# salute-developers/GigaAM

Hardware: AMD Instinct MI355X
Metric: RTFx v2_ctc batch32x20s (log-mel + encoder + greedy decode) (higher is better)
Workload: dtype f32 (GEMMs: 3-term split on fp16 MFMA, fp32 accumulate)

## Files before the change

### gigaam_amd/_lib.py

```python
from __future__ import annotations

import ctypes as C
import os
from typing import Optional

_HERE = os.path.dirname(os.path.abspath(__file__))
LIB_NAME = "libgigaam_hip.so"
LIB_PATH = os.path.join(_HERE, LIB_NAME)

SUBS_CONV2D, SUBS_CONV1D = 0, 1
ATT_ROTARY, ATT_REL_POS = 0, 1
NORM_BATCH, NORM_LAYER = 0, 1
HEAD_NONE, HEAD_CTC, HEAD_RNNT, HEAD_EMO = 0, 1, 2, 3
DTYPE_F32, DTYPE_F16, DTYPE_BF16, DTYPE_F64, DTYPE_I64 = 0, 1, 2, 3, 4
GEMM_F32, GEMM_F16X3, GEMM_F16 = 0, 1, 2
PF_CLASSES = ["gemm", "conv2", "attn", "norm", "convmod", "stem", "frontend", "decode", "misc", "align_bt", "align_out"]


class GamConfig(C.Structure):
    _fields_ = [(n, C.c_int32) for n in (
        "sample_rate", "n_mels", "hop_length", "win_length", "n_fft", "center",
        "feat_in", "n_layers", "d_model", "subsampling", "subs_kernel_size", "subsampling_factor",
        "ff_expansion_factor", "self_attention_model", "n_heads", "pos_emb_max_len",
        "conv_norm_type", "conv_kernel_size",
        "head_type", "num_classes", "pred_hidden", "pred_rnn_layers", "joint_hidden",
    )]


_P = C.c_void_p
SIGNATURES = {
    "gam_abi_version": (C.c_int, []),
    "gam_create": (C.c_int, [C.POINTER(GamConfig), C.c_int, C.POINTER(_P)]),
    "gam_destroy": (None, [_P]),
    "gam_set_weight": (C.c_int, [_P, C.c_char_p, _P, C.c_int, C.POINTER(C.c_int64), C.c_int]),
    "gam_finalize": (C.c_int, [_P]),
    "gam_feat_frames": (C.c_int64, [_P, C.c_int64]),
    "gam_enc_frames": (C.c_int64, [_P, C.c_int64]),
    "gam_frontend": (C.c_int, [_P, _P, _P, C.c_int, C.c_int64, _P, _P, _P]),
    "gam_encode": (C.c_int, [_P, _P, _P, C.c_int, C.c_int64, _P, _P, _P]),
    "gam_encode_ex": (C.c_int, [_P, _P, _P, C.c_int, C.c_int64, _P, _P, C.c_int, _P, _P]),
    "gam_encode_varlen": (C.c_int, [_P, _P, _P, C.POINTER(C.c_int64), C.c_int, C.c_int64, _P, _P, C.c_int, _P, _P]),
    "gam_last_encode_rows": (C.c_int, [_P, C.POINTER(C.c_int)]),
    "gam_ctc_head": (C.c_int, [_P, _P, C.c_int, C.c_int64, _P, _P]),
    "gam_ctc_greedy": (C.c_int, [_P, _P, _P, C.c_int, C.c_int64, _P, _P, _P, _P]),
    "gam_ctc_align": (C.c_int, [_P, _P, _P, C.c_int, C.c_int64, _P, _P, C.c_int, _P, _P, _P, _P, _P, _P, _P]),
    "gam_op_ctc_align": (C.c_int, [_P, _P, _P, C.c_int, C.c_int64, C.c_int, _P, _P, C.c_int, _P, _P, _P, _P, _P, _P, _P]),
    "gam_op_ctc_align_long": (C.c_int, [_P, _P, C.c_int64, C.c_int, _P, C.c_int, _P, _P, _P, _P, _P, _P, _P]),
    "gam_set_ctc_align_workspace": (C.c_int, [_P, C.c_int64]),
    "gam_tune_ctc_align_long": (C.c_int, [C.c_int, C.c_int]),
    "gam_ctc_kws": (C.c_int, [_P, _P, _P, C.c_int, C.c_int64, C.c_int, _P, _P, _P, _P, _P, _P]),
    "gam_op_ctc_kws": (C.c_int, [_P, _P, _P, C.c_int, C.c_int64, C.c_int, C.c_int, _P, _P, _P, _P, _P, _P]),
    "gam_set_keywords": (C.c_int, [_P, _P, _P, C.c_int, _P]),
    "gam_ctc_beam": (C.c_int, [_P, _P, _P, C.c_int, C.c_int64, C.c_int, _P, _P, _P, _P, _P, _P]),
    "gam_op_ctc_beam": (C.c_int, [_P, _P, _P, C.c_int, C.c_int64, C.c_int, C.c_int, _P, _P, _P, _P, _P, _P]),
    "gam_set_hotwords": (C.c_int, [_P, _P, _P, C.c_int, C.c_float]),
    "gam_set_lm": (C.c_int, [_P, _P, C.c_int, _P, C.c_int64, C.c_int, _P, C.c_int64, C.c_int, C.c_int, C.c_int, C.c_int, C.c_int,
                             C.c_float, C.c_float, C.c_float]),
    "gam_rnnt_greedy": (C.c_int, [_P, _P, _P, C.c_int, C.c_int64, C.c_int, _P, _P, _P, _P, _P, C.c_int, _P]),
    "gam_ctc_beam_nbest": (C.c_int, [_P, _P, _P, C.c_int, C.c_int64, C.c_int, C.c_int, _P, _P, _P, _P, _P, _P, _P]),
    "gam_op_ctc_beam_nbest": (C.c_int, [_P, _P, _P, C.c_int, C.c_int64, C.c_int, C.c_int, C.c_int, _P, _P, _P, _P, _P, _P, _P]),
    "gam_rnnt_beam_nbest": (C.c_int, [_P, _P, _P, C.c_int, C.c_int64, C.c_int, C.c_int, C.c_int, _P, _P, _P, _P, _P, _P, _P]),
    "gam_op_rnnt_beam_nbest": (C.c_int, [_P, _P, _P, C.c_int, C.c_int64, C.c_int, C.c_int, C.c_int, _P, _P, _P, _P, _P, _P, _P]),
    "gam_rnnt_beam": (C.c_int, [_P, _P, _P, C.c_int, C.c_int64, C.c_int, C.c_int, _P, _P, _P, _P, _P, _P]),
    "gam_op_rnnt_beam": (C.c_int, [_P, _P, _P, C.c_int, C.c_int64, C.c_int, C.c_int, _P, _P, _P, _P, _P, _P]),
    "gam_rnnt_align": (C.c_int, [_P, _P, _P, C.c_int, C.c_int64, _P, _P, C.c_int, _P, _P, _P, _P, _P]),
    "gam_op_rnnt_align": (C.c_int, [_P, _P, _P, C.c_int, C.c_int64, _P, _P, C.c_int, _P, _P, _P, _P, _P, _P]),
    "gam_op_rnnt_lattice_align": (C.c_int, [_P, _P, _P, C.c_int, C.c_int64, C.c_int, _P, _P, C.c_int, _P, _P, _P, _P, _P]),
    "gam_set_rnnt_align_workspace": (C.c_int, [_P, C.c_int64]),
    "gam_ctc_confidence": (C.c_int, [_P, _P, _P, C.c_int, C.c_int64, _P, _P, _P, C.c_int, C.c_int, C.c_int, _P, _P, _P, _P]),
    "gam_op_ctc_confidence": (C.c_int, [_P, _P, _P, C.c_int, C.c_int64, C.c_int, _P, _P, _P, C.c_int, C.c_int, C.c_int, _P, _P, _P, _P]),
    "gam_rnnt_confidence": (C.c_int, [_P, _P, _P, C.c_int, C.c_int64, _P, _P, _P, C.c_int, C.c_int, _P, _P, _P]),
    "gam_op_rnnt_confidence": (C.c_int, [_P, _P, _P, C.c_int, C.c_int64, _P, _P, _P, C.c_int, C.c_int, _P, _P, _P]),
    "gam_emo_probs": (C.c_int, [_P, _P, _P, C.c_int, C.c_int64, _P, _P]),
    "gam_rnnt_predict": (C.c_int, [_P, _P, _P, _P, C.c_int, _P, _P, _P, _P]),
    "gam_rnnt_joint": (C.c_int, [_P, _P, _P, C.c_int, C.c_int, C.c_int, _P, _P]),
    "gam_set_gemm_mode": (C.c_int, [_P, C.c_int]),
    "gam_get_gemm_mode": (C.c_int, [_P]),
    "gam_set_rnnt_cluster": (C.c_int, [_P, C.c_int]),
    "gam_get_rnnt_cluster": (C.c_int, [_P]),
    "gam_debug_buffer_hash": (C.c_int, [_P, C.c_int, C.POINTER(C.c_uint64), C.POINTER(C.c_int64)]),
    "gam_range_flag": (C.c_int, [_P, C.POINTER(C.c_int), _P]),
    "gam_range_flag_fetch": (C.c_int, [_P, _P, _P]),
    "gam_op_gemm": (C.c_int, [_P, _P, _P, _P, _P, C.c_int, C.c_int, C.c_int, C.c_int, _P]),
    "gam_op_attention": (C.c_int, [_P, _P, _P, _P, _P, _P, C.c_int, C.c_int, C.c_int, _P]),
    "gam_op_attention_ex": (C.c_int, [_P, _P, _P, _P, C.c_int64, _P, _P, _P, C.c_int, C.c_int, C.c_int, C.c_int, _P, _P, _P, _P]),
    "gam_tune_sp": (C.c_int, [C.c_int, C.c_int, C.c_int]),
    "gam_plan_sp": (C.c_int, [C.c_int, C.c_int, C.c_int, C.c_int, C.POINTER(C.c_int), C.POINTER(C.c_int), C.POINTER(C.c_int)]),
    "gam_plan_sp_ex": (C.c_int, [C.c_int, C.c_int, C.c_int, C.c_int, C.POINTER(C.c_int), C.POINTER(C.c_int), C.POINTER(C.c_int), C.POINTER(C.c_int)]),
    "gam_tune_sp_stages": (C.c_int, [C.c_int]),
    "gam_profile_enable": (C.c_int, [_P, C.c_int]),
    "gam_profile_pause": (C.c_int, [_P, C.c_int]),
    "gam_profile_read": (C.c_int, [_P, C.c_int, C.POINTER(C.c_double), C.POINTER(C.c_int64), C.POINTER(C.c_double)]),
    "gam_profile_read_bytes": (C.c_int, [_P, C.c_int, C.POINTER(C.c_double)]),
    "gam_last_error": (C.c_char_p, [_P]),
    "gam_comm_unique_id": (C.c_int, [C.c_char_p]),
    "gam_comm_create": (C.c_int, [C.c_char_p, C.c_int, C.c_int, C.c_int, C.POINTER(_P)]),
    "gam_comm_world": (C.c_int, [_P]),
    "gam_gather_ids": (C.c_int, [_P, _P, _P, _P, _P, C.c_int, C.c_int, _P, _P, _P, _P, _P]),
    "gam_comm_last_error": (C.c_char_p, [_P]),
    "gam_comm_destroy": (None, [_P]),
}

_lib: Optional[C.CDLL] = None


class GigaAMHipError(RuntimeError):
    pass


def load_library(path: Optional[str] = None) -> C.CDLL:
    global _lib
    if _lib is not None and path is None:
        return _lib
    p = path or os.environ.get("GIGAAM_HIP_LIB", LIB_PATH)
    if not os.path.exists(p):
        raise GigaAMHipError(
            f"{p} not found: the HIP extension is not built. Run `python -c 'import __graft_entry__ as g; g.build()'` "
            "(hipcc --offload-arch=gfx950). There is no CPU fallback.")
    lib = C.CDLL(p)
    for name, (res, args) in SIGNATURES.items():
        fn = getattr(lib, name)
        fn.restype = res
        fn.argtypes = args
    if lib.gam_abi_version() != 1:
        raise GigaAMHipError("libgigaam_hip.so ABI version mismatch")
    if path is None:
        _lib = lib
    return lib
```

### gigaam_amd/csrc/gam_api.hip

```cpp
#include <hip/hip_runtime.h>

#include <algorithm>
#include <cmath>
#include <cstdarg>
#include <cstdio>
#include <cstring>
#include <map>
#include <string>
#include <vector>

#include "../../include/gigaam_hip.h"
#include "gam_align.h"
#include "gam_align_long.h"
#include "gam_kws.h"
#include "gam_attn.h"
#include "gam_beam.h"
#include "gam_rnnt_beam.h"
#include "gam_attn16.h"
#include "gam_comm.h"
#include "gam_common.h"
#include "gam_convmod.h"
#include "gam_decode.h"
#include "gam_rnnt_align.h"
#include "gam_confidence.h"
// ... 2318 lines not shown
  if (int r = gemm(h, s, g, GAM_ACT_NONE, GAM_PF_DECODE)) return r;
  return rnnt_conf_launch(h, h->encp.p, enc_len, B, Tp, ids, frames, counts, cap, measure, conf, status, s);
}

int gam_op_rnnt_confidence(gam_handle* h, const float* encp, const int32_t* enc_len, int B, int64_t Tp, const int32_t* ids,
                           const int32_t* frames, const int32_t* counts, int cap, int measure, float* conf, int32_t* status, void* stream) {
  if (!h || !h->finalized) return fail(h, -1, "RNN-T head before gam_finalize");
  if (h->cfg.head_type != GAM_HEAD_RNNT || !h->has_head) return fail(h, -1, "model has no RNN-T head");
  hipStream_t s = (hipStream_t)stream;
  HIPCHK(h, hipSetDevice(h->device));
  DecodeScope ds(h, s);
  return rnnt_conf_launch(h, encp, enc_len, B, Tp, ids, frames, counts, cap, measure, conf, status, s);
}

int gam_rnnt_predict(gam_handle* h, const int32_t* labels, const float* h_in, const float* c_in, int B, float* g_out,
                     float* h_out, float* c_out, void* stream) {
  if (!h || !h->finalized) return fail(h, -1, "gam_rnnt_predict before gam_finalize");
  if (h->cfg.head_type != GAM_HEAD_RNNT || !h->has_head) return fail(h, -1, "model has no RNN-T head");
  if (B <= 0 || !g_out || !h_out || !c_out || (h_in == nullptr) != (c_in == nullptr)) return fail(h, -1, "bad gam_rnnt_predict arguments");
  HIPCHK(h, hipSetDevice(h->device));
  const gam_config& c = h->cfg;
  GamPredictArgs a;
  a.label = labels; a.h_in = h_in; a.c_in = c_in; a.g_out = g_out; a.h_out = h_out; a.c_out = c_out;
  a.gate_tab = h->lstm_tab; a.whh_t = h->lstm_whh_t; a.wih_x = h->lstm_wih_x; a.whh_x = h->lstm_whh_x; a.bias_x = h->lstm_bias_x;
  a.B = B; a.PH = c.pred_hidden; a.V = c.num_classes; a.L = c.pred_rnn_layers;
  hipStream_t s = (hipStream_t)stream;
  ProfScope ps(h, s, GAM_PF_DECODE, 0.0);
  hipLaunchKernelGGL(gam_rnnt_predict_kernel, dim3(B), dim3(256), (size_t)6 * c.pred_hidden * sizeof(float), s, a);
  HIPCHK(h, hipGetLastError());
  return 0;
}

int gam_rnnt_joint(gam_handle* h, const float* enc, const float* dec, int B, int T, int U, float* log_probs, void* stream) {
  if (!h || !h->finalized) return fail(h, -1, "gam_rnnt_joint before gam_finalize");
  if (h->cfg.head_type != GAM_HEAD_RNNT || !h->has_head) return fail(h, -1, "model has no RNN-T head");
  if (B <= 0 || T <= 0 || U <= 0 || !enc || !dec || !log_probs) return fail(h, -1, "bad gam_rnnt_joint arguments");
  HIPCHK(h, hipSetDevice(h->device));
  const gam_config& c = h->cfg;
  const int D = c.d_model, PH = c.pred_hidden, JH = c.joint_hidden, V = c.num_classes;
  const size_t rows = (size_t)B * T * U;
  if (rows * std::max(JH, V) > ((size_t)1 << 31)) return fail(h, -1, "gam_rnnt_joint: B x T x U = %zu rows is too large for one call", rows);
  hipStream_t s = (hipStream_t)stream;
  DecodeScope ds(h, s);
  if (int r = ensure(h, h->encp, (size_t)B * T * JH)) return r;
  if (int r = ensure(h, h->jp, (size_t)B * U * JH)) return r;
  if (int r = ensure(h, h->jz, rows * JH)) return r;
  if (int r = ensure(h, h->jl, rows * V)) return r;
  GamGemmArgs ge = gemm_args(enc, D, h->jn_enc_w, h->jn_enc_b, h->encp.p, JH, B * T, JH, D);
  if (int r = gemm(h, s, ge, GAM_ACT_NONE, GAM_PF_DECODE)) return r;
  GamGemmArgs gp = gemm_args(dec, PH, h->jn_pred_w, h->jn_pred_b, h->jp.p, JH, B * U, JH, PH);
  if (int r = gemm(h, s, gp, GAM_ACT_NONE, GAM_PF_DECODE)) return r;
  {
    ProfScope ps(h, s, GAM_PF_DECODE, (double)rows * JH * 4.0);
    const int grid = (int)std::min<size_t>((rows * JH + 255) / 256, 8192);
    hipLaunchKernelGGL(gam_joint_hidden_kernel, dim3(grid), dim3(256), 0, s, h->encp.p, h->jp.p, h->jz.p, B, T, U, JH);
    HIPCHK(h, hipGetLastError());
  }
  GamGemmArgs go = gemm_args(h->jz.p, JH, h->jn_out_w, h->jn_out_b, h->jl.p, V, (int)rows, V, JH);
  if (int r = gemm(h, s, go, GAM_ACT_NONE, GAM_PF_DECODE)) return r;
  ProfScope ps(h, s, GAM_PF_DECODE, (double)rows * V * 8.0);
  hipLaunchKernelGGL(gam_log_softmax_kernel, dim3(gam_cdiv((long)rows, 4)), dim3(256), 0, s, h->jl.p, log_probs, (int)rows, V);
  HIPCHK(h, hipGetLastError());
  return 0;
}

int gam_emo_probs(gam_handle* h, const float* encoded, const int32_t* enc_len, int B, int64_t Tp, float* probs,
                  void* stream) {
  if (!h) return -1;
  if (h->cfg.head_type != GAM_HEAD_EMO || !h->has_head) return fail(h, -1, "model has no emotion head");
  if (B <= 0 || Tp <= 0 || !encoded || !probs) return fail(h, -1, "bad emotion-head arguments");
  HIPCHK(h, hipSetDevice(h->device));
  hipStream_t s = (hipStream_t)stream;
  const int D = h->cfg.d_model, NC = h->cfg.num_classes;
  ProfScope ps(h, s, GAM_PF_DECODE, (double)B * D * Tp * 4.0);
  hipLaunchKernelGGL(gam_emo_head_kernel, dim3(B), dim3(256), (size_t)(D + NC) * sizeof(float), s, encoded, enc_len,
                     h->emo_w, h->emo_b, probs, D, (int)Tp, NC);
  HIPCHK(h, hipGetLastError());
  return 0;
}

int gam_op_gemm(gam_handle* h, const float* A, const float* W, const float* bias, float* C, int M, int N, int K, int act,
                void* stream) {
  if (!h) return -1;
  HIPCHK(h, hipSetDevice(h->device));
  GamGemmArgs g = gemm_args(A, K, W, bias, C, N, M, N, K);
  hipStream_t s = (hipStream_t)stream;
  if (!split_mode(h) || K % 32 != 0 || N % 4 != 0) return gemm(h, s, g, act);
  const size_t wn = (size_t)N * K, an = (size_t)M * K;
  W16 w16;
  if (int r = ensure(h, h->op_sp, wn + 64)) return r;
  hipLaunchKernelGGL(gam_to_sp32_kernel, dim3((int)std::min<size_t>((wn / 4 + 255) / 256, 4096)), dim3(256), 0, s, W,
                     (_Float16*)h->op_sp.p, wn / 4, (const float*)nullptr, K);
  w16.sp = (_Float16*)h->op_sp.p;
  if (int r = ensure(h, h->op_rs, (size_t)M + 64)) return r;
  hipLaunchKernelGGL(gam_rowscale_kernel, dim3(gam_cdiv(M, 4)), dim3(256), 0, s, A, h->op_rs.p, M, K, (long)K);
  g.a_rs = h->op_rs.p;
  if (int r = ensure(h, h->aplanes, an + 64)) return r;
  g.Asp = (const _Float16*)h->aplanes.p;
  g.a_fmt = (h->gemm_mode == GAM_GEMM_F16 && K % 64 == 0) ? 2 : 1;
  if (g.a_fmt == 2) {
    if (int r = ensure(h, h->op_planes, wn / 2 + 64)) return r;
    w16.h16 = (_Float16*)h->op_planes.p;
    hipLaunchKernelGGL(gam_to_h16_kernel, dim3((int)std::min<size_t>((wn / 4 + 255) / 256, 4096)), dim3(256), 0, s, W, w16.h16,
                       wn / 4, (const float*)nullptr, K);
    hipLaunchKernelGGL(gam_to_h16_kernel, dim3((int)std::min<size_t>((an / 4 + 255) / 256, 8192)), dim3(256), 0, s, A,
                       (_Float16*)h->aplanes.p, an / 4, (const float*)h->op_rs.p, K);
  } else {
    hipLaunchKernelGGL(gam_to_sp32_kernel, dim3((int)std::min<size_t>((an / 4 + 255) / 256, 8192)), dim3(256), 0, s, A,
                       (_Float16*)h->aplanes.p, an / 4, (const float*)h->op_rs.p, K);
  }
  return gemm(h, s, g, act, GAM_PF_GEMM, &w16);
}

int gam_op_attention(gam_handle* h, const float* q, const float* k, const float* v, float* ctx, const int32_t* lens, int B,
                     int T, int H, void* stream) {
  if (!h) return -1;
  if (B <= 0 || T <= 0 || H <= 0) return fail(h, -1, "bad attention shape");
  HIPCHK(h, hipSetDevice(h->device));
  GamAttnArgs at;
  memset(&at, 0, sizeof at);
  const int D = H * GAM_ATT_DK;
  at.q = q; at.k = k; at.v = v; at.ctx = ctx; at.lens = lens;
  at.B = B; at.Ta = T; at.Tv = T; at.H = H; at.ldq = D; at.ldv = D; at.ldo = D;
  at.scale = 1.0f / sqrtf((float)GAM_ATT_DK);
  hipError_t e = gam_launch_attn_mode(at, GAM_ATT_DK, split_mode(h), (hipStream_t)stream, h->gemm_mode == GAM_GEMM_F16 ? 1 : 3, h->ncu);
  if (e != hipSuccess) return fail(h, -2, "attention launch: %s", hipGetErrorString(e));
  return 0;
}

int gam_op_attention_ex(gam_handle* h, const float* q, const float* k, const float* v, int64_t ldq, float* ctx, const int32_t* lens,
                        const int32_t* cu, int B, int Ta, int Tv, int H, const float* pbuf, const float* pos_u, const float* pos_v,
                        void* stream) {
  if (!h) return -1;
  const int D = H * GAM_ATT_DK;
  if (B <= 0 || Ta <= 0 || Tv <= 0 || H <= 0) return fail(h, -1, "bad attention shape");
  if (cu == nullptr && Tv > Ta) return fail(h, -1, "attention: Tv %d > Ta %d in the padded layout", Tv, Ta);
  if (ldq < D || ldq % 4 != 0) return fail(h, -1, "attention: row stride %ld (H*48 = %d, multiple of 4)", (long)ldq, D);
  if (pbuf != nullptr && (pos_u == nullptr || pos_v == nullptr)) return fail(h, -1, "attention: pbuf without pos_u / pos_v");
  auto al16 = [](const void* p) { return (reinterpret_cast<uintptr_t>(p) & 15) == 0; };
  if (!al16(q) || !al16(k) || !al16(v) || !al16(ctx) || (pbuf && (!al16(pbuf) || !al16(pos_u) || !al16(pos_v))))
    return fail(h, -1, "attention: operands must be 16-byte aligned");
  HIPCHK(h, hipSetDevice(h->device));
  GamAttnArgs at;
  memset(&at, 0, sizeof at);
  at.q = q; at.k = k; at.v = v; at.ctx = ctx; at.lens = lens; at.cu = cu;
  at.B = B; at.Ta = Ta; at.Tv = Tv; at.H = H; at.ldq = ldq; at.ldv = ldq; at.ldo = D;
  at.scale = 1.0f / sqrtf((float)GAM_ATT_DK);
  at.pbuf = pbuf; at.pos_u = pos_u; at.pos_v = pos_v; at.ldp = D;
  hipError_t e = gam_launch_attn_mode(at, GAM_ATT_DK, split_mode(h), (hipStream_t)stream, h->gemm_mode == GAM_GEMM_F16 ? 1 : 3, h->ncu);
  if (e != hipSuccess) return fail(h, -2, "attention launch: %s", hipGetErrorString(e));
  return 0;
}

int gam_set_gemm_mode(gam_handle* h, int mode) {
  if (!h || (mode != GAM_GEMM_F32 && mode != GAM_GEMM_F16X3 && mode != GAM_GEMM_F16)) return fail(h, -1, "unknown GEMM mode %d", mode);
  h->gemm_mode = mode;
  return 0;
}

int gam_get_gemm_mode(const gam_handle* h) { return h ? h->gemm_mode : -1; }

int gam_debug_buffer_hash(gam_handle* h, int which, uint64_t* hash_out, int64_t* floats_out) {
  if (!h || !hash_out) return -1;
  const DevBuf* b = which == 0 ? &h->tok : which == 1 ? &h->encp : which == 2 ? &h->rnnt_x : which == 3 ? &h->logits : nullptr;
  if (!b) return fail(h, -1, "no such buffer %d", which);
  HIPCHK(h, hipSetDevice(h->device));
  HIPCHK(h, hipDeviceSynchronize());
  std::vector<uint32_t> host(b->cap);
  if (b->cap) HIPCHK(h, hipMemcpy(host.data(), b->p, b->cap * sizeof(float), hipMemcpyDeviceToHost));
  uint64_t x = 1469598103934665603ull;
  for (uint32_t v : host) { x ^= v; x *= 1099511628211ull; }
  *hash_out = x;
  if (floats_out) *floats_out = (int64_t)b->cap;
  return 0;
}

int gam_set_rnnt_cluster(gam_handle* h, int workgroups_per_utterance) {
  if (!h) return -1;
  if (workgroups_per_utterance < -1 || workgroups_per_utterance > 8) return fail(h, -1, "cluster size %d outside -1 (auto) .. 8", workgroups_per_utterance);
  h->rnnt_cluster = workgroups_per_utterance;
  return 0;
}

int gam_get_rnnt_cluster(gam_handle* h) { return h ? h->rnnt_cluster : -2; }

int gam_last_encode_rows(gam_handle* h, int* rows_padded) {
  if (!h) return -1;
  if (rows_padded) *rows_padded = h->last_rows_padded;
  return h->last_rows;
}

int gam_range_flag(gam_handle* h, int* flag_host, void* stream) {
  if (!h || !flag_host) return -1;
  if (!h->finalized) return fail(h, -1, "gam_range_flag before gam_finalize");
  HIPCHK(h, hipSetDevice(h->device));
  hipStream_t s = (hipStream_t)stream;
  HIPCHK(h, hipMemcpyAsync(flag_host, h->range_flag, sizeof(int), hipMemcpyDeviceToHost, s));
  HIPCHK(h, hipMemsetAsync(h->range_flag, 0, sizeof(int), s));
  HIPCHK(h, hipStreamSynchronize(s));
  return 0;
}

int gam_range_flag_fetch(gam_handle* h, int32_t* flag_dev, void* stream) {
  if (!h || !flag_dev) return -1;
  if (!h->finalized) return fail(h, -1, "gam_range_flag_fetch before gam_finalize");
  HIPCHK(h, hipSetDevice(h->device));
  hipStream_t s = (hipStream_t)stream;
  HIPCHK(h, hipMemcpyAsync(flag_dev, h->range_flag, sizeof(int), hipMemcpyDeviceToDevice, s));
  HIPCHK(h, hipMemsetAsync(h->range_flag, 0, sizeof(int), s));
  return 0;
}

int gam_plan_sp(int M, int N, int K, int n_cu, int* mt, int* nw, int* splitk) {
  if (M <= 0 || N <= 0 || K <= 0 || K % 32 != 0 || !mt || !nw || !splitk) return -1;
  const GamSpPlan p = gam_gemm_sp_plan(M, N, K, 0, n_cu > 0 ? n_cu : 256);
  *mt = p.mt; *nw = p.nw; *splitk = p.s;
  return 0;
}

int gam_tune_sp(int mt, int nw, int splitk) {
  GamSpForce& f = gam_sp_force();
  f.mt = mt; f.nw = nw; f.s = splitk;
  return 0;
}

int gam_tune_sp_stages(int stages) {
  if (stages != 0 && stages != 2 && stages != 3) return -1;
  gam_sp_force().ns = stages;
  return 0;
}

int gam_plan_sp_ex(int M, int N, int K, int n_cu, int* mt, int* nw, int* splitk, int* stages) {
  if (M <= 0 || N <= 0 || K <= 0 || K % 32 != 0 || !mt || !nw || !splitk || !stages) return -1;
  const GamSpPlan p = gam_gemm_sp_plan(M, N, K, 0, n_cu > 0 ? n_cu : 256);
  *mt = p.mt; *nw = p.nw; *splitk = p.s; *stages = p.ns;
  return 0;
}

int gam_profile_enable(gam_handle* h, int on) {
  if (!h) return -1;
  h->prof_on = on;
  h->prof_used = 0;
  for (int i = 0; i < GAM_PF_NCLASS; ++i) { h->prof_work[i] = 0; h->prof_launches[i] = 0; h->prof_bytes[i] = 0; }
  return 0;
}

int gam_profile_pause(gam_handle* h, int on) {
  if (!h) return -1;
  h->prof_on = on;
  return 0;
}

int gam_profile_read_bytes(gam_handle* h, int cls, double* bytes) {
  if (!h || cls < 0 || cls >= GAM_PF_NCLASS || !bytes) return -1;
  *bytes = h->prof_bytes[cls];
  return 0;
}

int gam_profile_read(gam_handle* h, int cls, double* ms, int64_t* launches, double* work) {
  if (!h || cls < 0 || cls >= GAM_PF_NCLASS) return -1;
  double tot = 0;
  for (size_t i = 0; i < h->prof_used; ++i) {
    ProfEvent& e = h->prof_events[i];
    if (e.cls != cls) continue;
    HIPCHK(h, hipEventSynchronize(e.b));
    float t = 0;
    HIPCHK(h, hipEventElapsedTime(&t, e.a, e.b));
    tot += t;
  }
  if (ms) *ms = tot;
  if (launches) *launches = h->prof_launches[cls];
  if (work) *work = h->prof_work[cls];
  return 0;
}

}
```

### gigaam_amd/csrc/gam_attn16.h

```cpp
#pragma once
#include "gam_attn.h"

#define GAM_A16_KLD 56
#define GAM_A16_VLD 72

__device__ __forceinline__ void gam_split8(const float (&v)[8], gam_half8& hi, gam_half8& lo) {
  gam_u32x4 h, l;
#pragma unroll
  for (int i = 0; i < 4; ++i) {
    unsigned hh, ll;
    gam_split2(v[2 * i], v[2 * i + 1], hh, ll);
    h[i] = hh;
    l[i] = ll;
  }
  hi = __builtin_bit_cast(gam_half8, h);
  lo = __builtin_bit_cast(gam_half8, l);
}

#ifndef GAM_ATT_NJ
#define GAM_ATT_NJ 2
#endif
#ifndef GAM_ATT_PV_TERMS
#define GAM_ATT_PV_TERMS 3
#endif
// ... 157 lines not shown
        kl32 = *reinterpret_cast<const gam_half8*>(&Kl[ko + 8 * lg]);
        kl16 = *reinterpret_cast<const gam_half4*>(&Kl[ko + 32 + 4 * lg]);
      }
#pragma unroll
      for (int j = 0; j < NJ; ++j) {
        f32x4 s = (f32x4){0.f, 0.f, 0.f, 0.f};
        f32x4 s16 = (f32x4){0.f, 0.f, 0.f, 0.f};
        if (LO) {
          s = __builtin_amdgcn_mfma_f32_16x16x32_f16(kl32, qh32[j], s, 0, 0, 0);
          s16 = __builtin_amdgcn_mfma_f32_16x16x16f16(kl16, qh16[j], s16, 0, 0, 0);
          s = __builtin_amdgcn_mfma_f32_16x16x32_f16(kh32, ql32[j], s, 0, 0, 0);
          s16 = __builtin_amdgcn_mfma_f32_16x16x16f16(kh16, ql16[j], s16, 0, 0, 0);
        }
        s = __builtin_amdgcn_mfma_f32_16x16x32_f16(kh32, qh32[j], s, 0, 0, 0);
        s16 = __builtin_amdgcn_mfma_f32_16x16x16f16(kh16, qh16[j], s16, 0, 0, 0);
        s += s16;
        st[kb][j] = s;
      }
    }

    if (REL) {
      float* gw = Gs + wave * (80 * 17);
#pragma unroll
      for (int j = 0; j < NJ; ++j) {
        const int rlo = (qw0 + j * 16) - kt0 - 63 + (a.Tv - 1);
#pragma unroll
        for (int mt = 0; mt < 5; ++mt) {
          int prow = rlo + mt * 16 + li;
          prow = prow < 0 ? 0 : (prow > 2 * a.Tv - 2 ? 2 * a.Tv - 2 : prow);
          const float* pp = a.pbuf + (size_t)prow * a.ldp + h * DK;
          const float4 p0 = *reinterpret_cast<const float4*>(pp + 8 * lg);
          const float4 p1 = *reinterpret_cast<const float4*>(pp + 8 * lg + 4);
          const float4 p2 = *reinterpret_cast<const float4*>(pp + 32 + 4 * lg);
          const float p8[8] = {p0.x, p0.y, p0.z, p0.w, p1.x, p1.y, p1.z, p1.w};
          gam_half8 ph32, pl32;
          gam_half4 ph16, pl16;
          gam_split8(p8, ph32, pl32);
          gam_split4((f32x4){p2.x, p2.y, p2.z, p2.w}, ph16, pl16);
          f32x4 g = (f32x4){0.f, 0.f, 0.f, 0.f};
          f32x4 g16 = (f32x4){0.f, 0.f, 0.f, 0.f};
          if (LO) {
            g = __builtin_amdgcn_mfma_f32_16x16x32_f16(pl32, gh32[j], g, 0, 0, 0);
            g16 = __builtin_amdgcn_mfma_f32_16x16x16f16(pl16, gh16[j], g16, 0, 0, 0);
            g = __builtin_amdgcn_mfma_f32_16x16x32_f16(ph32, gl32[j], g, 0, 0, 0);
            g16 = __builtin_amdgcn_mfma_f32_16x16x16f16(ph16, gl16[j], g16, 0, 0, 0);
          }
          g = __builtin_amdgcn_mfma_f32_16x16x32_f16(ph32, gh32[j], g, 0, 0, 0);
          g16 = __builtin_amdgcn_mfma_f32_16x16x16f16(ph16, gh16[j], g16, 0, 0, 0);
          g += g16;
#pragma unroll
          for (int r = 0; r < 4; ++r) gw[(mt * 16 + lg * 4 + r) * 17 + li] = g[r];
        }
        __syncthreads();
#pragma unroll
        for (int kb = 0; kb < 4; ++kb)
#pragma unroll
          for (int r = 0; r < 4; ++r) st[kb][j][r] += gw[(li - (kb * 16 + lg * 4 + r) + 63) * 17 + li];
        __syncthreads();
      }
    }

    const bool full_tile = kt0 + GAM_ATT_KT <= klen;
#pragma unroll
    for (int j = 0; j < NJ; ++j) {
      float mx = -INFINITY;
      if (full_tile) {
#pragma unroll
        for (int kb = 0; kb < 4; ++kb)
#pragma unroll
          for (int r = 0; r < 4; ++r) mx = fmaxf(mx, st[kb][j][r]);
      } else {
#pragma unroll
        for (int kb = 0; kb < 4; ++kb)
#pragma unroll
          for (int r = 0; r < 4; ++r) {
            const int key = kt0 + kb * 16 + lg * 4 + r;
            float s = st[kb][j][r];
            s = key < klen ? s : -INFINITY;
            st[kb][j][r] = s;
            mx = fmaxf(mx, s);
          }
      }
      mx = fmaxf(mx, __shfl_xor(mx, 16, 64));
      mx = fmaxf(mx, __shfl_xor(mx, 32, 64));
      const float mnew = fmaxf(mrun[j], mx);
      const float alpha = __builtin_amdgcn_exp2f(mrun[j] - mnew);
      mrun[j] = mnew;
      float ps = 0.f;
#pragma unroll
      for (int kb = 0; kb < 4; ++kb)
#pragma unroll
        for (int r = 0; r < 4; ++r) {
          const float p = __builtin_amdgcn_exp2f(st[kb][j][r] - mnew);
          st[kb][j][r] = p;
          ps += p;
        }
      lsum[j] = lsum[j] * alpha + ps;
#pragma unroll
      for (int d = 0; d < 3; ++d) {
        o[d][j][0] *= alpha; o[d][j][1] *= alpha;
        o[d][j][2] *= alpha; o[d][j][3] *= alpha;
      }
    }

#pragma unroll
    for (int c = 0; c < 2; ++c) {
      gam_half8 ph[NJ], pl[NJ];
#pragma unroll
      for (int j = 0; j < NJ; ++j) {
        const float p8[8] = {st[2 * c][j][0], st[2 * c][j][1], st[2 * c][j][2], st[2 * c][j][3],
                             st[2 * c + 1][j][0], st[2 * c + 1][j][1], st[2 * c + 1][j][2], st[2 * c + 1][j][3]};
        gam_split8(p8, ph[j], pl[j]);
      }
#pragma unroll
      for (int d = 0; d < 3; ++d) {
        const int vo = (d * 16 + li) * GAM_A16_VLD + 4 * lg;
        const gam_half4 vh0 = *reinterpret_cast<const gam_half4*>(&Vh[vo + (2 * c) * 16]);
        const gam_half4 vh1 = *reinterpret_cast<const gam_half4*>(&Vh[vo + (2 * c + 1) * 16]);
        const gam_half8 vh = {vh0[0], vh0[1], vh0[2], vh0[3], vh1[0], vh1[1], vh1[2], vh1[3]};
        gam_half8 vl = vh;
        if (LO) {
          const gam_half4 vl0 = *reinterpret_cast<const gam_half4*>(&Vl[vo + (2 * c) * 16]);
          const gam_half4 vl1 = *reinterpret_cast<const gam_half4*>(&Vl[vo + (2 * c + 1) * 16]);
          vl = (gam_half8){vl0[0], vl0[1], vl0[2], vl0[3], vl1[0], vl1[1], vl1[2], vl1[3]};
        }
#pragma unroll
        for (int j = 0; j < NJ; ++j) {
          if (LO) {
            o[d][j] = __builtin_amdgcn_mfma_f32_16x16x32_f16(vl, ph[j], o[d][j], 0, 0, 0);
            if (GAM_ATT_PV_TERMS == 3) o[d][j] = __builtin_amdgcn_mfma_f32_16x16x32_f16(vh, pl[j], o[d][j], 0, 0, 0);
          }
          o[d][j] = __builtin_amdgcn_mfma_f32_16x16x32_f16(vh, ph[j], o[d][j], 0, 0, 0);
        }
      }
    }
    __syncthreads();
  }

#pragma unroll
  for (int j = 0; j < NJ; ++j) {
    float l = lsum[j];
    l += __shfl_xor(l, 16, 64);
    l += __shfl_xor(l, 32, 64);
    const float inv = l > 0.f ? 1.0f / l : 0.f;
    if (qrow[j] < rlim) {
#pragma unroll
      for (int d = 0; d < 3; ++d)
        gam_store4(a.ctx, (size_t)(rowbase + qrow[j]) * a.ldo, h * DK + 4 * lg + 16 * d, o[d][j][0] * inv, o[d][j][1] * inv,
                   o[d][j][2] * inv, o[d][j][3] * inv, a.ctx_split);
    }
  }
}

static inline hipError_t gam_launch_attn_mode(const GamAttnArgs& a, int dk, bool split, hipStream_t s, int terms = 3, int ncu = 256) {
  if (!split) return gam_launch_attn(a, dk, s);
  if (dk != GAM_ATT_DK) return hipErrorInvalidValue;
  static const int nj_env = []() { const char* e = getenv("GAM_ATT_NJ_SMALL"); return e ? atoi(e) : -1; }();
  const long wgs128 = (long)gam_cdiv(a.Ta, 64 * GAM_ATT_NJ) * a.H * a.B;
  const bool small = GAM_ATT_NJ == 2 && (nj_env < 0 ? wgs128 < (long)ncu : (nj_env > 0 && wgs128 < (long)nj_env * ncu));
  const bool rel = a.pbuf != nullptr;
#define GAM_ATT_GO(REL_, T_, NJ_)                                                                      \
  hipLaunchKernelGGL((gam_attn_f16x3_kernel<REL_, T_, NJ_>), dim3(gam_cdiv(a.Ta, 64 * NJ_), a.H, a.B), dim3(256), 0, s, a)
  if (small) {
    if (terms == 1) { if (rel) GAM_ATT_GO(true, 1, 1); else GAM_ATT_GO(false, 1, 1); }
    else { if (rel) GAM_ATT_GO(true, 3, 1); else GAM_ATT_GO(false, 3, 1); }
  } else {
    if (terms == 1) { if (rel) GAM_ATT_GO(true, 1, GAM_ATT_NJ); else GAM_ATT_GO(false, 1, GAM_ATT_NJ); }
    else { if (rel) GAM_ATT_GO(true, 3, GAM_ATT_NJ); else GAM_ATT_GO(false, 3, GAM_ATT_NJ); }
  }
#undef GAM_ATT_GO
  return hipGetLastError();
}
```

### include/gigaam_hip.h

```cpp
#ifndef GIGAAM_HIP_H
#define GIGAAM_HIP_H

#include <stdint.h>

#ifdef __cplusplus
extern "C" {
#endif

#define GAM_ABI_VERSION 1

typedef struct gam_handle gam_handle;

enum { GAM_SUBS_CONV2D = 0, GAM_SUBS_CONV1D = 1 };
enum { GAM_ATT_ROTARY = 0, GAM_ATT_REL_POS = 1 };
enum { GAM_NORM_BATCH = 0, GAM_NORM_LAYER = 1 };
enum { GAM_HEAD_NONE = 0, GAM_HEAD_CTC = 1, GAM_HEAD_RNNT = 2, GAM_HEAD_EMO = 3 };
enum { GAM_DTYPE_F32 = 0, GAM_DTYPE_F16 = 1, GAM_DTYPE_BF16 = 2, GAM_DTYPE_F64 = 3, GAM_DTYPE_I64 = 4 };

typedef struct gam_config {
  int32_t sample_rate, n_mels, hop_length, win_length, n_fft, center;
  int32_t feat_in, n_layers, d_model, subsampling, subs_kernel_size, subsampling_factor;
  int32_t ff_expansion_factor, self_attention_model, n_heads, pos_emb_max_len;
  int32_t conv_norm_type, conv_kernel_size;
  int32_t head_type, num_classes, pred_hidden, pred_rnn_layers, joint_hidden;
} gam_config;

int gam_abi_version(void);

int gam_create(const gam_config* cfg, int device_id, gam_handle** out);
void gam_destroy(gam_handle* h);

int gam_set_weight(gam_handle* h, const char* key, const void* host_ptr, int dtype,
                   const int64_t* shape, int ndim);

int gam_finalize(gam_handle* h);

int64_t gam_feat_frames(const gam_handle* h, int64_t n_samples);
int64_t gam_enc_frames(const gam_handle* h, int64_t n_feat_frames);

int gam_frontend(gam_handle* h, const float* wav, const int64_t* wav_len, int B, int64_t L,
                 float* feat, int64_t* feat_len, void* stream);

int gam_encode(gam_handle* h, const float* feat, const int64_t* feat_len, int B, int64_t T,
               float* encoded, int32_t* enc_len, void* stream);

int gam_encode_ex(gam_handle* h, const float* feat, const int64_t* feat_len, int B, int64_t T,
                  float* encoded, int32_t* enc_len, int n_layers_run, float* tokens_out, void* stream);

int gam_encode_varlen(gam_handle* h, const float* feat, const int64_t* feat_len, const int64_t* feat_len_host, int B, int64_t T,
                      float* encoded, int32_t* enc_len, int n_layers_run, float* tokens_out, void* stream);

int gam_last_encode_rows(gam_handle* h, int* rows_padded);

int gam_ctc_head(gam_handle* h, const float* encoded, int B, int64_t Tp, float* log_probs, void* stream);

int gam_ctc_greedy(gam_handle* h, const float* encoded, const int32_t* enc_len, int B, int64_t Tp,
                   int32_t* ids, int32_t* frames, int32_t* counts, void* stream);

int gam_ctc_align(gam_handle* h, const float* encoded, const int32_t* enc_len, int B, int64_t Tp, const int32_t* targets,
                  const int32_t* target_len, int Umax, int32_t* frame_labels, int32_t* tok_first, int32_t* tok_last, float* score,
                  float* loglik, int32_t* status, void* stream);
int gam_op_ctc_align(gam_handle* h, const float* log_probs, const int32_t* enc_len, int B, int64_t Tp, int V, const int32_t* targets,
                     const int32_t* target_len, int Umax, int32_t* frame_labels, int32_t* tok_first, int32_t* tok_last, float* score,
                     float* loglik, int32_t* status, void* stream);

int gam_op_ctc_align_long(gam_handle* h, const float* log_probs, int64_t T, int V, const int32_t* targets, int U, int32_t* frame_labels,
                          int32_t* tok_first, int32_t* tok_last, double* score, double* loglik, int32_t* status, void* stream);
int gam_set_ctc_align_workspace(gam_handle* h, int64_t bytes);
int gam_tune_ctc_align_long(int sb, int tt);

int gam_ctc_kws(gam_handle* h, const float* encoded, const int32_t* enc_len, int B, int64_t Tp, int max_hits, int32_t* hit_frames,
                float* hit_score, int32_t* n_hits, float* dense_score, int32_t* dense_start, void* stream);
int gam_op_ctc_kws(gam_handle* h, const float* log_probs, const int32_t* enc_len, int B, int64_t Tp, int V, int max_hits,
                   int32_t* hit_frames, float* hit_score, int32_t* n_hits, float* dense_score, int32_t* dense_start, void* stream);
int gam_set_keywords(gam_handle* h, const int32_t* tokens, const int32_t* offsets, int n_keywords, const float* min_score);

int gam_ctc_beam(gam_handle* h, const float* encoded, const int32_t* enc_len, int B, int64_t Tp, int W, int32_t* ids, int32_t* frames,
                 int32_t* counts, float* score, float* logp, void* stream);
int gam_op_ctc_beam(gam_handle* h, const float* log_probs, const int32_t* enc_len, int B, int64_t Tp, int V, int W, int32_t* ids,
                    int32_t* frames, int32_t* counts, float* score, float* logp, void* stream);
int gam_ctc_beam_nbest(gam_handle* h, const float* encoded, const int32_t* enc_len, int B, int64_t Tp, int W, int N, int32_t* ids,
                       int32_t* frames, int32_t* counts, float* score, float* logp, int32_t* n_hyp, void* stream);
int gam_op_ctc_beam_nbest(gam_handle* h, const float* log_probs, const int32_t* enc_len, int B, int64_t Tp, int V, int W, int N,
                          int32_t* ids, int32_t* frames, int32_t* counts, float* score, float* logp, int32_t* n_hyp, void* stream);
int gam_set_hotwords(gam_handle* h, const int32_t* tokens, const int32_t* offsets, int n_phrases, float boost);
int gam_set_lm(gam_handle* h, const int32_t* token_class, int V, const void* word_table, int64_t word_slots, int word_probe,
               const void* ngram_table, int64_t ngram_slots, int ngram_probe, int order, int bos, int eos, int unk, float unk_logp,
               float weight, float word_bonus);

int gam_rnnt_greedy(gam_handle* h, const float* encoded, const int32_t* enc_len, int B, int64_t Tp,
                    int max_symbols, int32_t* ids, int32_t* frames, int32_t* counts,
                    float* logits_dump, int32_t* dump_count, int dump_cap, void* stream);

int gam_rnnt_beam(gam_handle* h, const float* encoded, const int32_t* enc_len, int B, int64_t Tp, int W, int max_symbols, int32_t* ids,
                  int32_t* frames, int32_t* counts, float* score, float* logp, void* stream);
int gam_op_rnnt_beam(gam_handle* h, const float* encp, const int32_t* enc_len, int B, int64_t Tp, int W, int max_symbols, int32_t* ids,
                     int32_t* frames, int32_t* counts, float* score, float* logp, void* stream);

int gam_rnnt_beam_nbest(gam_handle* h, const float* encoded, const int32_t* enc_len, int B, int64_t Tp, int W, int max_symbols, int N,
                        int32_t* ids, int32_t* frames, int32_t* counts, float* score, float* logp, int32_t* n_hyp, void* stream);
int gam_op_rnnt_beam_nbest(gam_handle* h, const float* encp, const int32_t* enc_len, int B, int64_t Tp, int W, int max_symbols, int N,
                           int32_t* ids, int32_t* frames, int32_t* counts, float* score, float* logp, int32_t* n_hyp, void* stream);

int gam_rnnt_align(gam_handle* h, const float* encoded, const int32_t* enc_len, int B, int64_t Tp, const int32_t* targets,
                   const int32_t* target_len, int Umax, int32_t* tok_frame, float* score, float* loglik, int32_t* status, void* stream);
int gam_op_rnnt_align(gam_handle* h, const float* encp, const int32_t* enc_len, int B, int64_t Tp, const int32_t* targets,
                      const int32_t* target_len, int Umax, int32_t* tok_frame, float* score, float* loglik, int32_t* status,
                      float* lattice_out, void* stream);
int gam_op_rnnt_lattice_align(gam_handle* h, const float* lattice, const int32_t* enc_len, int B, int64_t Tp, int V, const int32_t* targets,
                              const int32_t* target_len, int Umax, int32_t* tok_frame, float* score, float* loglik, int32_t* status,
                              void* stream);
int gam_set_rnnt_align_workspace(gam_handle* h, int64_t bytes);

int gam_ctc_confidence(gam_handle* h, const float* encoded, const int32_t* enc_len, int B, int64_t Tp, const int32_t* ids,
                       const int32_t* frames, const int32_t* counts, int cap, int measure, int agg, float* conf, int32_t* span,
                       int32_t* status, void* stream);
int gam_op_ctc_confidence(gam_handle* h, const float* log_probs, const int32_t* enc_len, int B, int64_t Tp, int V, const int32_t* ids,
                          const int32_t* frames, const int32_t* counts, int cap, int measure, int agg, float* conf, int32_t* span,
                          int32_t* status, void* stream);
int gam_rnnt_confidence(gam_handle* h, const float* encoded, const int32_t* enc_len, int B, int64_t Tp, const int32_t* ids,
                        const int32_t* frames, const int32_t* counts, int cap, int measure, float* conf, int32_t* status, void* stream);
int gam_op_rnnt_confidence(gam_handle* h, const float* encp, const int32_t* enc_len, int B, int64_t Tp, const int32_t* ids,
                           const int32_t* frames, const int32_t* counts, int cap, int measure, float* conf, int32_t* status, void* stream);

int gam_set_rnnt_cluster(gam_handle* h, int workgroups_per_utterance);
int gam_get_rnnt_cluster(gam_handle* h);

int gam_debug_buffer_hash(gam_handle* h, int which, uint64_t* hash_out, int64_t* floats_out);

int gam_rnnt_predict(gam_handle* h, const int32_t* labels, const float* h_in, const float* c_in, int B, float* g_out,
                     float* h_out, float* c_out, void* stream);
int gam_rnnt_joint(gam_handle* h, const float* enc, const float* dec, int B, int T, int U, float* log_probs, void* stream);

int gam_emo_probs(gam_handle* h, const float* encoded, const int32_t* enc_len, int B, int64_t Tp, float* probs,
                  void* stream);

enum { GAM_GEMM_F32 = 0, GAM_GEMM_F16X3 = 1, GAM_GEMM_F16 = 2 };
int gam_set_gemm_mode(gam_handle* h, int mode);
int gam_range_flag(gam_handle* h, int* flag_host, void* stream);
int gam_range_flag_fetch(gam_handle* h, int32_t* flag_dev, void* stream);
int gam_get_gemm_mode(const gam_handle* h);

int gam_op_gemm(gam_handle* h, const float* A, const float* W, const float* bias, float* C,
                int M, int N, int K, int act, void* stream);

int gam_op_attention(gam_handle* h, const float* q, const float* k, const float* v, float* ctx,
                     const int32_t* lens, int B, int T, int H, void* stream);
int gam_op_attention_ex(gam_handle* h, const float* q, const float* k, const float* v, int64_t ldq, float* ctx,
                        const int32_t* lens, const int32_t* cu, int B, int Ta, int Tv, int H, const float* pbuf,
                        const float* pos_u, const float* pos_v, void* stream);

int gam_tune_sp(int mt, int nw, int splitk);
int gam_plan_sp(int M, int N, int K, int n_cu, int* mt, int* nw, int* splitk);
int gam_plan_sp_ex(int M, int N, int K, int n_cu, int* mt, int* nw, int* splitk, int* stages);
int gam_tune_sp_stages(int stages);

enum { GAM_PF_GEMM = 0, GAM_PF_CONV2 = 1, GAM_PF_ATTN = 2, GAM_PF_NORM = 3, GAM_PF_CONVMOD = 4,
       GAM_PF_STEM = 5, GAM_PF_FRONTEND = 6, GAM_PF_DECODE = 7, GAM_PF_MISC = 8,
       GAM_PF_ALIGN_BT = 9, GAM_PF_ALIGN_OUT = 10,
       GAM_PF_NCLASS = 11 };
int gam_profile_enable(gam_handle* h, int on);
int gam_profile_read(gam_handle* h, int cls, double* ms, int64_t* launches, double* work);
int gam_profile_pause(gam_handle* h, int on);
int gam_profile_read_bytes(gam_handle* h, int cls, double* bytes);

typedef struct gam_comm gam_comm;
#define GAM_COMM_ID_BYTES 128
int gam_comm_unique_id(char id_out[GAM_COMM_ID_BYTES]);
int gam_comm_create(const char id[GAM_COMM_ID_BYTES], int rank, int world, int device_id, gam_comm** out);
int gam_comm_world(const gam_comm* c);
int gam_gather_ids(gam_comm* c, const int32_t* index, const int32_t* counts, const int32_t* ids, const int32_t* frames,
                   int rows, int cap, int32_t* all_index, int32_t* all_counts, int32_t* all_ids, int32_t* all_frames,
                   void* stream);
const char* gam_comm_last_error(const gam_comm* c);
void gam_comm_destroy(gam_comm* c);

const char* gam_last_error(const gam_handle* h);

#ifdef __cplusplus
}
#endif
#endif
```

Before: 20670.

## Add wide 512-thread attention kernel sharing double-buffered K/V tiles across eight waves

Adds a flash-attention variant in which each workgroup runs eight waves over a larger block of query rows. K/V tiles are prefetched into registers and staged into double-buffered LDS as split fp16 hi/lo planes, so each loaded tile serves more query rows and the next tile's load overlaps compute. The launcher picks this kernel for non-relative-position attention when enough workgroups exist to fill the CUs, and a GAM_ATT_WG environment variable can force the choice. The trade-off is fewer, larger workgroups with higher register and LDS pressure, which may lower occupancy. A debug getter reports which shape was last launched.

```diff
diff --git a/gigaam_amd/_lib.py b/gigaam_amd/_lib.py
--- a/gigaam_amd/_lib.py
+++ b/gigaam_amd/_lib.py
@@ -79,6 +79,7 @@
     "gam_set_rnnt_cluster": (C.c_int, [_P, C.c_int]),
     "gam_get_rnnt_cluster": (C.c_int, [_P]),
     "gam_debug_buffer_hash": (C.c_int, [_P, C.c_int, C.POINTER(C.c_uint64), C.POINTER(C.c_int64)]),
+    "gam_debug_attn_shape": (C.c_int, []),
     "gam_range_flag": (C.c_int, [_P, C.POINTER(C.c_int), _P]),
     "gam_range_flag_fetch": (C.c_int, [_P, _P, _P]),
     "gam_op_gemm": (C.c_int, [_P, _P, _P, _P, _P, C.c_int, C.c_int, C.c_int, C.c_int, _P]),
diff --git a/gigaam_amd/csrc/gam_api.hip b/gigaam_amd/csrc/gam_api.hip
--- a/gigaam_amd/csrc/gam_api.hip
+++ b/gigaam_amd/csrc/gam_api.hip
@@ -2494,6 +2494,8 @@
   return 0;
 }
 
+int gam_debug_attn_shape(void) { return gam_attn_last_wg; }
+
 int gam_set_gemm_mode(gam_handle* h, int mode) {
   if (!h || (mode != GAM_GEMM_F32 && mode != GAM_GEMM_F16X3 && mode != GAM_GEMM_F16)) return fail(h, -1, "unknown GEMM mode %d", mode);
   h->gemm_mode = mode;
diff --git a/gigaam_amd/csrc/gam_attn16.h b/gigaam_amd/csrc/gam_attn16.h
--- a/gigaam_amd/csrc/gam_attn16.h
+++ b/gigaam_amd/csrc/gam_attn16.h
@@ -333,6 +333,269 @@
   }
 }
 
+template <int TERMS, int NJ, int NW>
+__global__ __launch_bounds__(64 * NW, 2) void gam_attn_f16x3_wide_kernel(GamAttnArgs a) {
+  constexpr bool LO = TERMS == 3;
+  constexpr int DK = GAM_ATT_DK, NT = 64 * NW;
+  constexpr int KP = GAM_ATT_KT * GAM_A16_KLD, VP = DK * GAM_A16_VLD;
+  constexpr int BUF = (LO ? 2 : 1) * (KP + VP);
+  constexpr int KIT = (GAM_ATT_KT * 12 + NT - 1) / NT, VIT = (32 * 12 + NT - 1) / NT;
+  static_assert(GAM_ATT_KT == 64 && DK == 48 && KP % 8 == 0 && VP % 8 == 0, "plane offsets must keep the 16-byte alignment");
+  a.scale *= 1.44269504088896341f;
+  __shared__ __attribute__((aligned(16))) _Float16 sm[2 * BUF];
+  const int tid = threadIdx.x, lane = tid & 63, wave = tid >> 6;
+  const int li = lane & 15, lg = lane >> 4;
+  const int b = blockIdx.z, h = blockIdx.y;
+  int klen = a.Tv;
+  if (a.lens != nullptr) { const int l = a.lens[b]; klen = l < a.Tv ? l : a.Tv; }
+  const GamRows ur = gam_rows(a.cu, b, a.Ta, klen);
+  if ((int)blockIdx.x * (16 * NJ * NW) >= ur.lim) return;
+  const size_t rowbase = ur.base;
+  const int rlim = ur.lim;
+  const int qw0 = blockIdx.x * (16 * NJ * NW) + wave * (16 * NJ);
+  const bool active = qw0 < rlim;
+
+  gam_half8 qh32[NJ], ql32[NJ];
+  gam_half4 qh16[NJ], ql16[NJ];
+  int qrow[NJ];
+#pragma unroll
+  for (int j = 0; j < NJ; ++j) {
+    const int qi = qw0 + j * 16 + li;
+    qrow[j] = qi;
+    const int qc = qi < rlim ? qi : rlim - 1;
+    const float* qp = a.q + (rowbase + qc) * a.ldq + h * DK;
+    const float4 q0 = *reinterpret_cast<const float4*>(qp + 8 * lg);
+    const float4 q1 = *reinterpret_cast<const float4*>(qp + 8 * lg + 4);
+    const float4 q2 = *reinterpret_cast<const float4*>(qp + 32 + 4 * lg);
+    float v8[8] = {q0.x, q0.y, q0.z, q0.w, q1.x, q1.y, q1.z, q1.w};
+#pragma unroll
+    for (int e = 0; e < 8; ++e) v8[e] *= a.scale;
+    gam_split8(v8, qh32[j], ql32[j]);
+    gam_split4((f32x4){q2.x * a.scale, q2.y * a.scale, q2.z * a.scale, q2.w * a.scale}, qh16[j], ql16[j]);
+  }
+
+  f32x4 o[3][NJ];
+#pragma unroll
+  for (int d = 0; d < 3; ++d)
+#pragma unroll
+    for (int j = 0; j < NJ; ++j) o[d][j] = (f32x4){0.f, 0.f, 0.f, 0.f};
+  float mrun[NJ], lsum[NJ];
+#pragma unroll
+  for (int j = 0; j < NJ; ++j) { mrun[j] = -INFINITY; lsum[j] = 0.f; }
+
+  float4 kreg[KIT], vreg[VIT][2];
+  auto fetch_tile = [&](int kt0) {
+#pragma unroll
+    for (int i = 0; i < KIT; ++i) {
+      const int idx = tid + i * NT;
+      if (KIT * NT == GAM_ATT_KT * 12 || idx < GAM_ATT_KT * 12) {
+        const int kr = idx / 12, c4 = (idx - kr * 12) * 4;
+        int key = kt0 + kr;
+        key = key < rlim ? key : rlim - 1;
+        kreg[i] = *reinterpret_cast<const float4*>(a.k + (rowbase + key) * a.ldq + h * DK + c4);
+      }
+    }
+#pragma unroll
+    for (int i = 0; i < VIT; ++i) {
+      const int it = tid + i * NT;
+      if (VIT * NT == 32 * 12 || it < 32 * 12) {
+        const int kp = it / 12, c4 = (it - kp * 12) * 4;
+        int k0 = kt0 + 2 * kp, k1 = k0 + 1;
+        k0 = k0 < rlim ? k0 : rlim - 1;
+        k1 = k1 < rlim ? k1 : rlim - 1;
+        vreg[i][0] = *reinterpret_cast<const float4*>(a.v + (rowbase + k0) * a.ldv + h * DK + c4);
+        vreg[i][1] = *reinterpret_cast<const float4*>(a.v + (rowbase + k1) * a.ldv + h * DK + c4);
+      }
+    }
+  };
+  auto stage_tile = [&](int buf) {
+    _Float16* Kh = sm + buf * BUF;
+    _Float16* Vh = Kh + KP;
+    _Float16* Kl = LO ? Vh + VP : Kh;
+    _Float16* Vl = LO ? Kl + KP : Vh;
+#pragma unroll
+    for (int i = 0; i < KIT; ++i) {
+      const int idx = tid + i * NT;
+      if (KIT * NT == GAM_ATT_KT * 12 || idx < GAM_ATT_KT * 12) {
+        const int kr = idx / 12, c4 = (idx - kr * 12) * 4;
+        gam_half4 hi, lo;
+        gam_split4((f32x4){kreg[i].x, kreg[i].y, kreg[i].z, kreg[i].w}, hi, lo);
+        *reinterpret_cast<gam_half4*>(&Kh[kr * GAM_A16_KLD + c4]) = hi;
+        if (LO) *reinterpret_cast<gam_half4*>(&Kl[kr * GAM_A16_KLD + c4]) = lo;
+      }
+    }
+#pragma unroll
+    for (int i = 0; i < VIT; ++i) {
+      const int it = tid + i * NT;
+      if (VIT * NT == 32 * 12 || it < 32 * 12) {
+        const int kp = it / 12, c4 = (it - kp * 12) * 4;
+        gam_half4 h0, l0, h1, l1;
+        gam_split4((f32x4){vreg[i][0].x, vreg[i][0].y, vreg[i][0].z, vreg[i][0].w}, h0, l0);
+        gam_split4((f32x4){vreg[i][1].x, vreg[i][1].y, vreg[i][1].z, vreg[i][1].w}, h1, l1);
+        typedef _Float16 half2_t __attribute__((ext_vector_type(2)));
+#pragma unroll
+        for (int e = 0; e < 4; ++e) {
+          *reinterpret_cast<half2_t*>(&Vh[(c4 + e) * GAM_A16_VLD + 2 * kp]) = (half2_t){h0[e], h1[e]};
+          if (LO) *reinterpret_cast<half2_t*>(&Vl[(c4 + e) * GAM_A16_VLD + 2 * kp]) = (half2_t){l0[e], l1[e]};
+        }
+      }
+    }
+  };
+
+  if (klen > 0) {
+    fetch_tile(0);
+    stage_tile(0);
+    if (GAM_ATT_KT < klen) fetch_tile(GAM_ATT_KT);
+    __syncthreads();
+  }
+
+  int cur = 0;
+  for (int kt0 = 0; kt0 < klen; kt0 += GAM_ATT_KT, cur ^= 1) {
+    const _Float16* Kh = sm + cur * BUF;
+    const _Float16* Vh = Kh + KP;
+    const _Float16* Kl = LO ? Vh + VP : Kh;
+    const _Float16* Vl = LO ? Kl + KP : Vh;
+    const bool more = kt0 + GAM_ATT_KT < klen;
+
+    f32x4 st[4][NJ];
+    if (active) {
+#pragma unroll
+      for (int kb = 0; kb < 4; ++kb) {
+        const int ko = (kb * 16 + li) * GAM_A16_KLD;
+        const gam_half8 kh32 = *reinterpret_cast<const gam_half8*>(&Kh[ko + 8 * lg]);
+        const gam_half4 kh16 = *reinterpret_cast<const gam_half4*>(&Kh[ko + 32 + 4 * lg]);
+        gam_half8 kl32 = kh32;
+        gam_half4 kl16 = kh16;
+        if (LO) {
+          kl32 = *reinterpret_cast<const gam_half8*>(&Kl[ko + 8 * lg]);
+          kl16 = *reinterpret_cast<const gam_half4*>(&Kl[ko + 32 + 4 * lg]);
+        }
+#pragma unroll
+        for (int j = 0; j < NJ; ++j) {
+          f32x4 s = (f32x4){0.f, 0.f, 0.f, 0.f};
+          f32x4 s16 = (f32x4){0.f, 0.f, 0.f, 0.f};
+          if (LO) {
+            s = __builtin_amdgcn_mfma_f32_16x16x32_f16(kl32, qh32[j], s, 0, 0, 0);
+            s16 = __builtin_amdgcn_mfma_f32_16x16x16f16(kl16, qh16[j], s16, 0, 0, 0);
+            s = __builtin_amdgcn_mfma_f32_16x16x32_f16(kh32, ql32[j], s, 0, 0, 0);
+            s16 = __builtin_amdgcn_mfma_f32_16x16x16f16(kh16, ql16[j], s16, 0, 0, 0);
+          }
+          s = __builtin_amdgcn_mfma_f32_16x16x32_f16(kh32, qh32[j], s, 0, 0, 0);
+          s16 = __builtin_amdgcn_mfma_f32_16x16x16f16(kh16, qh16[j], s16, 0, 0, 0);
+          s += s16;
+          st[kb][j] = s;
+        }
+      }
+    }
+
+    if (more) {
+      stage_tile(cur ^ 1);
+      if (kt0 + 2 * GAM_ATT_KT < klen) fetch_tile(kt0 + 2 * GAM_ATT_KT);
+    }
+
+    if (active) {
+      const bool full_tile = kt0 + GAM_ATT_KT <= klen;
+      float alpha[NJ];
+      bool rescale = false;
+#pragma unroll
+      for (int j = 0; j < NJ; ++j) {
+        float mx = -INFINITY;
+        if (full_tile) {
+#pragma unroll
+          for (int kb = 0; kb < 4; ++kb)
+#pragma unroll
+            for (int r = 0; r < 4; ++r) mx = fmaxf(mx, st[kb][j][r]);
+        } else {
+#pragma unroll
+          for (int kb = 0; kb < 4; ++kb)
+#pragma unroll
+            for (int r = 0; r < 4; ++r) {
+              const int key = kt0 + kb * 16 + lg * 4 + r;
+              float s = st[kb][j][r];
+              s = key < klen ? s : -INFINITY;
+              st[kb][j][r] = s;
+              mx = fmaxf(mx, s);
+            }
+        }
+        mx = fmaxf(mx, __shfl_xor(mx, 16, 64));
+        mx = fmaxf(mx, __shfl_xor(mx, 32, 64));
+        const float mnew = fmaxf(mrun[j], mx);
+        alpha[j] = __builtin_amdgcn_exp2f(mrun[j] - mnew);
+        mrun[j] = mnew;
+        rescale = rescale || alpha[j] != 1.0f;
+        float ps = 0.f;
+#pragma unroll
+        for (int kb = 0; kb < 4; ++kb)
+#pragma unroll
+          for (int r = 0; r < 4; ++r) {
+            const float p = __builtin_amdgcn_exp2f(st[kb][j][r] - mnew);
+            st[kb][j][r] = p;
+            ps += p;
+          }
+        lsum[j] = lsum[j] * alpha[j] + ps;
+      }
+      if (__any(rescale)) {
+#pragma unroll
+        for (int j = 0; j < NJ; ++j)
+#pragma unroll
+          for (int d = 0; d < 3; ++d) {
+            o[d][j][0] *= alpha[j]; o[d][j][1] *= alpha[j];
+            o[d][j][2] *= alpha[j]; o[d][j][3] *= alpha[j];
+          }
+      }
+
+#pragma unroll
+      for (int c = 0; c < 2; ++c) {
+        gam_half8 ph[NJ], pl[NJ];
+#pragma unroll
+        for (int j = 0; j < NJ; ++j) {
+          const float p8[8] = {st[2 * c][j][0], st[2 * c][j][1], st[2 * c][j][2], st[2 * c][j][3],
+                               st[2 * c + 1][j][0], st[2 * c + 1][j][1], st[2 * c + 1][j][2], st[2 * c + 1][j][3]};
+          gam_split8(p8, ph[j], pl[j]);
+        }
+#pragma unroll
+        for (int d = 0; d < 3; ++d) {
+          const int vo = (d * 16 + li) * GAM_A16_VLD + 4 * lg;
+          const gam_half4 vh0 = *reinterpret_cast<const gam_half4*>(&Vh[vo + (2 * c) * 16]);
+          const gam_half4 vh1 = *reinterpret_cast<const gam_half4*>(&Vh[vo + (2 * c + 1) * 16]);
+          const gam_half8 vh = {vh0[0], vh0[1], vh0[2], vh0[3], vh1[0], vh1[1], vh1[2], vh1[3]};
+          gam_half8 vl = vh;
+          if (LO) {
+            const gam_half4 vl0 = *reinterpret_cast<const gam_half4*>(&Vl[vo + (2 * c) * 16]);
+            const gam_half4 vl1 = *reinterpret_cast<const gam_half4*>(&Vl[vo + (2 * c + 1) * 16]);
+            vl = (gam_half8){vl0[0], vl0[1], vl0[2], vl0[3], vl1[0], vl1[1], vl1[2], vl1[3]};
+          }
+#pragma unroll
+          for (int j = 0; j < NJ; ++j) {
+            if (LO) {
+              o[d][j] = __builtin_amdgcn_mfma_f32_16x16x32_f16(vl, ph[j], o[d][j], 0, 0, 0);
+              if (GAM_ATT_PV_TERMS == 3) o[d][j] = __builtin_amdgcn_mfma_f32_16x16x32_f16(vh, pl[j], o[d][j], 0, 0, 0);
+            }
+            o[d][j] = __builtin_amdgcn_mfma_f32_16x16x32_f16(vh, ph[j], o[d][j], 0, 0, 0);
+          }
+        }
+      }
+    }
+    __syncthreads();
+  }
+
+#pragma unroll
+  for (int j = 0; j < NJ; ++j) {
+    float l = lsum[j];
+    l += __shfl_xor(l, 16, 64);
+    l += __shfl_xor(l, 32, 64);
+    const float inv = l > 0.f ? 1.0f / l : 0.f;
+    if (qrow[j] < rlim) {
+#pragma unroll
+      for (int d = 0; d < 3; ++d)
+        gam_store4(a.ctx, (size_t)(rowbase + qrow[j]) * a.ldo, h * DK + 4 * lg + 16 * d, o[d][j][0] * inv, o[d][j][1] * inv,
+                   o[d][j][2] * inv, o[d][j][3] * inv, a.ctx_split);
+    }
+  }
+}
+
+static int gam_attn_last_wg = 0;
+
 static inline hipError_t gam_launch_attn_mode(const GamAttnArgs& a, int dk, bool split, hipStream_t s, int terms = 3, int ncu = 256) {
   if (!split) return gam_launch_attn(a, dk, s);
   if (dk != GAM_ATT_DK) return hipErrorInvalidValue;
@@ -340,6 +603,17 @@
   const long wgs128 = (long)gam_cdiv(a.Ta, 64 * GAM_ATT_NJ) * a.H * a.B;
   const bool small = GAM_ATT_NJ == 2 && (nj_env < 0 ? wgs128 < (long)ncu : (nj_env > 0 && wgs128 < (long)nj_env * ncu));
   const bool rel = a.pbuf != nullptr;
+  const char* wg_env = getenv("GAM_ATT_WG");
+  const int wg_force = wg_env ? atoi(wg_env) : 0;
+  const bool wide = GAM_ATT_NJ == 2 && !rel && wg_force != 128 &&
+                    (wg_force == 256 || (!small && (long)gam_cdiv(a.Ta, 128 * GAM_ATT_NJ) * a.H * a.B >= (long)ncu));
+  gam_attn_last_wg = wide ? 256 : (small ? 64 : 64 * GAM_ATT_NJ);
+  if (wide) {
+    const dim3 grid(gam_cdiv(a.Ta, 128 * GAM_ATT_NJ), a.H, a.B);
+    if (terms == 1) hipLaunchKernelGGL((gam_attn_f16x3_wide_kernel<1, GAM_ATT_NJ, 8>), grid, dim3(512), 0, s, a);
+    else hipLaunchKernelGGL((gam_attn_f16x3_wide_kernel<3, GAM_ATT_NJ, 8>), grid, dim3(512), 0, s, a);
+    return hipGetLastError();
+  }
 #define GAM_ATT_GO(REL_, T_, NJ_)                                                                      \
   hipLaunchKernelGGL((gam_attn_f16x3_kernel<REL_, T_, NJ_>), dim3(gam_cdiv(a.Ta, 64 * NJ_), a.H, a.B), dim3(256), 0, s, a)
   if (small) {
diff --git a/include/gigaam_hip.h b/include/gigaam_hip.h
--- a/include/gigaam_hip.h
+++ b/include/gigaam_hip.h
@@ -128,6 +128,8 @@
 
 int gam_debug_buffer_hash(gam_handle* h, int which, uint64_t* hash_out, int64_t* floats_out);
 
+int gam_debug_attn_shape(void);
+
 int gam_rnnt_predict(gam_handle* h, const int32_t* labels, const float* h_in, const float* c_in, int B, float* g_out,
                      float* h_out, float* c_out, void* stream);
 int gam_rnnt_joint(gam_handle* h, const float* enc, const float* dec, int B, int T, int U, float* log_probs, void* stream);
```

Result: slower. 20370 (-1.4%).
